# minhtrangvy/distributed_bitcoin_minter

Measured on AMD Instinct MI355X. Metric: GH/s (SHA-256 "msg nonce" min-search) at 1/2/4/8 MI355X; % of int32 VALU peak, higher is better.
Workload: dtype u32

## Files before the change

distributed_bitcoin_minter_amd/csrc/bm_kernels.hpp:

```cpp
#pragma once
#include <hip/hip_runtime.h>

#include <cstdint>
#include <type_traits>

#include "bm_common.h"
#include "bm_sha256.hpp"

namespace bm {

#define BM_DEV __device__ __forceinline__

template <int B, int E, class F>
BM_DEV void static_for(F&& f) {
    if constexpr (B < E) {
        f(std::integral_constant<int, B>{});
        static_for<B + 1, E>(f);
    }
}

BM_DEV uint32_t rotr(uint32_t x, uint32_t n) { return __builtin_amdgcn_alignbit(x, x, n); }

BM_DEV uint32_t xor3(uint32_t a, uint32_t b, uint32_t c) {
    if (__builtin_constant_p(a) && __builtin_constant_p(b) && __builtin_constant_p(c)) return a ^ b ^ c;
    return __builtin_amdgcn_bitop3_b32(a, b, c, 0x96);
}
BM_DEV uint32_t ch(uint32_t e, uint32_t f, uint32_t g) {
    if (__builtin_constant_p(e) && __builtin_constant_p(f) && __builtin_constant_p(g)) return (e & f) ^ (~e & g);
    return __builtin_amdgcn_bitop3_b32(e, f, g, 0xCA);
}
BM_DEV uint32_t maj(uint32_t a, uint32_t b, uint32_t c) {
    if (__builtin_constant_p(a) && __builtin_constant_p(b) && __builtin_constant_p(c))
        return (a & b) ^ (a & c) ^ (b & c);
    return __builtin_amdgcn_bitop3_b32(a, b, c, 0xE8);
}
BM_DEV uint32_t bsig0(uint32_t a) { return xor3(rotr(a, 2), rotr(a, 13), rotr(a, 22)); }
BM_DEV uint32_t bsig1(uint32_t e) { return xor3(rotr(e, 6), rotr(e, 11), rotr(e, 25)); }
BM_DEV uint32_t ssig0(uint32_t x) { return xor3(rotr(x, 7), rotr(x, 18), x >> 3); }
BM_DEV uint32_t ssig1(uint32_t x) { return xor3(rotr(x, 17), rotr(x, 19), x >> 10); }

template <int T>
BM_DEV void sha_round(uint32_t (&s)[8], uint32_t w) {
    uint32_t& a = s[(0 - T) & 7];
    uint32_t& b = s[(1 - T) & 7];
    uint32_t& c = s[(2 - T) & 7];
    uint32_t& d = s[(3 - T) & 7];
    uint32_t& e = s[(4 - T) & 7];
    uint32_t& f = s[(5 - T) & 7];
    uint32_t& g = s[(6 - T) & 7];
    uint32_t& h = s[(7 - T) & 7];
    const uint32_t t1 = h + bsig1(e) + ch(e, f, g) + (kK256[T] + w);
    d += t1;
    h = t1 + bsig0(a) + maj(a, b, c);
}

#ifndef BM_PAD_ADD3S
#define BM_PAD_ADD3S 1
#endif

BM_DEV uint32_t add3_sgpr(uint32_t a, uint32_t s, uint32_t b) {
    uint32_t r;
    asm("v_add3_u32 %0, %1, %2, %3" : "=v"(r) : "v"(a), "s"(s), "v"(b));
    return r;
}

template <int T, bool KW_SGPR = false>
BM_DEV void sha_round_kw(uint32_t (&s)[8], uint32_t kw) {
    uint32_t& a = s[(0 - T) & 7];
    uint32_t& b = s[(1 - T) & 7];
    uint32_t& c = s[(2 - T) & 7];
    uint32_t& d = s[(3 - T) & 7];
    uint32_t& e = s[(4 - T) & 7];
    uint32_t& f = s[(5 - T) & 7];
    uint32_t& g = s[(6 - T) & 7];
    uint32_t& h = s[(7 - T) & 7];
    uint32_t t1;
    if constexpr (KW_SGPR && BM_PAD_ADD3S)
        t1 = add3_sgpr(h, kw, ch(e, f, g)) + bsig1(e);
    else
        t1 = h + bsig1(e) + ch(e, f, g) + kw;
    d += t1;
    h = t1 + bsig0(a) + maj(a, b, c);
}

template <int R0, int R1>
BM_DEV void sha_rounds(uint32_t (&s)[8], uint32_t (&w)[16]) {
    static_for<R0, R1>([&](auto I) {
        constexpr int t = decltype(I)::value;
        if constexpr (t >= 16)
            w[t & 15] = ssig1(w[(t - 2) & 15]) + w[(t - 7) & 15] + ssig0(w[(t - 15) & 15]) + w[t & 15];
        sha_round<t>(s, w[t & 15]);
    });
}

BM_DEV uint32_t ssig0_uniform(uint32_t x) {
    return ((x >> 7) | (x << 25)) ^ ((x >> 18) | (x << 14)) ^ (x >> 3);
}

#ifndef BM_PIN
#define BM_PIN 1
#endif

BM_DEV uint32_t ssig0_salu(uint32_t x) {
    uint32_t r, t0, t1, t2;
    asm("s_lshr_b32 %1, %4, 7\n\t"
        "s_lshl_b32 %2, %4, 25\n\t"
        "s_or_b32 %1, %1, %2\n\t"
        "s_lshr_b32 %2, %4, 18\n\t"
        "s_lshl_b32 %3, %4, 14\n\t"
        "s_or_b32 %2, %2, %3\n\t"
        "s_xor_b32 %1, %1, %2\n\t"
        "s_lshr_b32 %2, %4, 3\n\t"
        "s_xor_b32 %0, %1, %2"
        : "=s"(r), "=&s"(t0), "=&s"(t1), "=&s"(t2)
        : "s"(x)
        : "scc");
    return r;
}

BM_DEV uint32_t vgpr_copy(uint32_t x) {
    uint32_t r;
    asm("v_mov_b32 %0, %1" : "=v"(r) : "s"(x));
    return r;
}

template <int R0, int V>
BM_DEV uint32_t sha_rounds_h0(uint32_t (&s)[8], uint32_t (&w)[16], uint32_t s0v, uint32_t h0_add) {
    static_assert(R0 <= V && V >= 1 && V <= 15, "varying word");
    static_for<R0, 63>([&](auto I) {
        constexpr int t = decltype(I)::value;
        if constexpr (t >= 16) {
            uint32_t s0;
            if constexpr (t - 15 == V)
                s0 = s0v;
            else
                s0 = ssig0(w[(t - 15) & 15]);
            w[t & 15] = ssig1(w[(t - 2) & 15]) + w[(t - 7) & 15] + s0 + w[t & 15];
        }
        sha_round<t>(s, w[t & 15]);
    });
    w[15] = ssig1(w[13]) + w[8] + ssig0(w[0]) + w[15];
    const uint32_t a = s[1], b = s[2], c = s[3], e = s[5], f = s[6], g = s[7], h = s[0];
    const uint32_t t1 = h + bsig1(e) + ch(e, f, g) + (kK256[63] + h0_add) + w[15];
    return t1 + bsig0(a) + maj(a, b, c);
}

BM_DEV void sha_compress(uint32_t (&st)[8], uint32_t (&w)[16]) {
    uint32_t s[8];
#pragma unroll
    for (int i = 0; i < 8; ++i) s[i] = st[i];
    sha_rounds<0, 64>(s, w);
#pragma unroll
    for (int i = 0; i < 8; ++i) st[i] += s[i];
}

template <int P, bool PADB>
constexpr int64_t tail_word(int k) {
    constexpr int LW = P / 4;
    if (k == LW + 1 && (P % 4) == 3 && P != 63) return 0x80000000ll;
    if (!PADB && k == 15) return -1;
    return 0;
}

template <int P, int NBV>
BM_DEV void add_task_digits(uint32_t (&W)[16 * NBV], uint64_t t, uint32_t ms, uint32_t nd) {
    uint64_t x = t;
    static_for<1, 20>([&](auto I) {
        constexpr int i = decltype(I)::value;
        constexpr int pos = 64 * (NBV - 1) + P - i;
        if constexpr (pos >= 0) {
            if (i >= (int)ms && i < (int)nd) {
                const uint64_t q = x / 10u;
                const uint32_t d = (uint32_t)(x - q * 10u);
                x = q;
                W[pos >> 2] += d << (8 * (3 - (pos & 3)));
            }
        }
    });
}

BM_DEV bool lex_less(uint64_t h1, uint64_t n1, uint64_t h2, uint64_t n2) {
    return h1 < h2 || (h1 == h2 && n1 < n2);
}

template <int XOR>
BM_DEV uint64_t swizzle_xor_u64(uint64_t v) {
    constexpr int pat = (XOR << 10) | 0x1F;
    const uint32_t lo = (uint32_t)__builtin_amdgcn_ds_swizzle((int)(uint32_t)v, pat);
    const uint32_t hi = (uint32_t)__builtin_amdgcn_ds_swizzle((int)(uint32_t)(v >> 32), pat);
    return ((uint64_t)hi << 32) | lo;
}

BM_DEV uint64_t readlane_u64(uint64_t v, int lane) {
    const uint32_t lo = (uint32_t)__builtin_amdgcn_readlane((int)(uint32_t)v, lane);
    const uint32_t hi = (uint32_t)__builtin_amdgcn_readlane((int)(uint32_t)(v >> 32), lane);
    return ((uint64_t)hi << 32) | lo;
}

BM_DEV void wave_min(uint64_t& h, uint64_t& n) {
    static_for<0, 5>([&](auto I) {
        constexpr int x = 1 << decltype(I)::value;
        const uint64_t oh = swizzle_xor_u64<x>(h), on = swizzle_xor_u64<x>(n);
        if (lex_less(oh, on, h, n)) {
            h = oh;
            n = on;
        }
    });
    const uint64_t h0 = readlane_u64(h, 0), n0 = readlane_u64(n, 0);
    const uint64_t h1 = readlane_u64(h, 32), n1 = readlane_u64(n, 32);
    if (lex_less(h1, n1, h0, n0)) {
        h = h1;
        n = n1;
    } else {
        h = h0;
        n = n0;
    }
}

template <int NT>
BM_DEV bool block_min(uint64_t& h, uint64_t& n) {
    constexpr int NWAVE = NT / 64;
    __shared__ Partial sh[NWAVE];
    wave_min(h, n);
    const int wave = threadIdx.x >> 6;
    if ((threadIdx.x & 63) == 0) sh[wave] = Partial{h, n};
    __syncthreads();
    if (threadIdx.x == 0) {
#pragma unroll
        for (int i = 1; i < NWAVE; ++i)
            if (lex_less(sh[i].hash, sh[i].nonce, h, n)) {
                h = sh[i].hash;
                n = sh[i].nonce;
            }
        return true;
    }
    return false;
}

BM_DEV uint64_t readfirstlane_u64(uint64_t v) {
    const uint32_t lo = (uint32_t)__builtin_amdgcn_readfirstlane((int)(uint32_t)v);
    const uint32_t hi = (uint32_t)__builtin_amdgcn_readfirstlane((int)(uint32_t)(v >> 32));
    return ((uint64_t)hi << 32) | lo;
}

#ifndef BM_FOLD
#define BM_FOLD 1
#endif
#ifndef BM_WAVES_MAIN
#define BM_WAVES_MAIN 7
#endif
#ifndef BM_WAVES_PAD
#define BM_WAVES_PAD 5
#endif
#ifndef BM_WAVES_NBV2
#define BM_WAVES_NBV2 7
#endif
#ifndef BM_NBV2_TIGHT
#define BM_NBV2_TIGHT 1
#endif
constexpr bool nbv2_tight(int P) { return BM_NBV2_TIGHT && P == 4; }
constexpr int search_waves(int P, int NBV) {
    return (NBV == 1 && P >= 55) ? BM_WAVES_PAD
                                 : (NBV == 2 ? (nbv2_tight(P) ? 6 : BM_WAVES_NBV2) : BM_WAVES_MAIN);
}
#ifndef BM_LDS_BEST
#define BM_LDS_BEST 0
#endif
#ifndef BM_CLOCK_PROBE
#define BM_CLOCK_PROBE 0
#endif
constexpr int kClockSlot = 16;
#ifndef BM_KATTR
#define BM_KATTR __attribute__((amdgpu_waves_per_eu(search_waves(P, NBV), 8)))
#endif

template <int P, int NBV, int PADK, bool TGT = false, bool HITS = false>
BM_DEV void search_body(const SearchArgs& A, Partial* __restrict__ part, unsigned long long* __restrict__ counter,
                        uint64_t target = 0, unsigned long long* hit = nullptr, Partial* hit_buf = nullptr,
                        uint64_t hit_cap = 0) {
    static_assert(!(TGT || HITS) || PADK == -1, "target and hits modes run the generic kernels");
    static_assert(!(TGT && HITS), "one mode");
    static_assert(P >= 0 && P < 64 && (NBV == 1 || (NBV == 2 && P <= 18)), "layout");
    constexpr int LW = P / 4;
    constexpr int BOFF = 16 * (NBV - 1);
    constexpr bool PADB = (NBV == 1) && (P >= 55);
    constexpr bool PADC = PADK >= 0;
    static_assert(!PADC || (PADB && PADK <= kMaxPadPrefixBlocks), "PADK is a padding-block layout");
    constexpr bool TWOW = (P % 4 == 0) && (LW >= 1);
    constexpr bool kFold = BM_FOLD && !PADB && LW >= 1 && !(NBV == 1 && (P == 53 || P == 54)) &&
                           !(NBV == 2 && P >= 17);
    constexpr bool kPin = BM_PIN && kFold && !(NBV == 1 && P >= 48);

    constexpr uint32_t inc0 = 1u << (8 * (3 - P % 4));
    constexpr uint32_t inc1 = (P % 4) >= 1 ? 1u << (8 * (4 - P % 4)) : 0u;
    constexpr uint32_t inc2 = (P % 4) >= 2 ? 1u << (8 * (5 - P % 4)) : 0u;
    constexpr uint32_t inc3 = (P % 4) >= 3 ? 1u << (8 * (6 - P % 4)) : 0u;

    uint64_t best_h = ~0ull, best_n = ~0ull;
    uint32_t bh = 0xFFFFFFFFu;
    const uint32_t thi = (uint32_t)(target >> 32);
    (void)thi;
#if BM_LDS_BEST
    __shared__ uint64_t lbest_h[kBlock], lbest_n[kBlock];
    lbest_h[threadIdx.x] = ~0ull;
    lbest_n[threadIdx.x] = ~0ull;
#endif

    const uint32_t S = A.S;
    const uint32_t n_in = TWOW ? 10u : S;
    const uint32_t n_out = TWOW ? S / 10u : 1u;
    const uint32_t lane = threadIdx.x & 63;
    const uint64_t ntask = A.t_end - A.t0;
    const uint64_t chunk = 64ull * A.chunk_m;

    if (BM_CLOCK_PROBE && blockIdx.x == 0 && threadIdx.x == 0) {
        counter[kClockSlot + 0] = __builtin_amdgcn_s_memtime();
        counter[kClockSlot + 1] = __builtin_amdgcn_s_memrealtime();
    }
    for (;;) {
        uint64_t base = 0;
        if constexpr (TGT) {
            uint64_t seen = 0;
            if (lane == 0) {
                base = atomicAdd(counter, (unsigned long long)chunk);
                seen = __hip_atomic_load(hit, __ATOMIC_RELAXED, __HIP_MEMORY_SCOPE_AGENT);
            }
            base = readfirstlane_u64(base);
            if (base >= ntask) break;
            seen = readfirstlane_u64(seen);
            if (seen < A.nonce_base || seen - A.nonce_base < (A.t0 + base) * (uint64_t)S) break;
        } else {
            if (lane == 0) base = atomicAdd(counter, (unsigned long long)chunk);
            base = readfirstlane_u64(base);
            if (base >= ntask) break;
        }
        for (uint32_t i = 0; i < A.chunk_m; ++i) {
            const uint64_t tt = base + 64ull * i + lane;
            if (tt >= ntask) break;
            const uint64_t t = A.t0 + tt;

            uint32_t W[16 * NBV];
            static_for<0, 16 * NBV>([&](auto K) { W[decltype(K)::value] = A.tmpl[decltype(K)::value]; });
            add_task_digits<P, NBV>(W, t, A.ms, A.nd);

            uint32_t st[8];
#pragma unroll
            for (int q = 0; q < 8; ++q) st[q] = PADK == 0 ? kIV256[q] : A.mid[q];
            if constexpr (NBV == 2) {
                uint32_t wa[16];
#pragma unroll
                for (int k = 0; k < 16; ++k) wa[k] = W[k];
                sha_compress(st, wa);
            }

            uint32_t wb[16];
            static_for<0, 16>([&](auto K) {
                constexpr int k = decltype(K)::value;
                if constexpr (k <= LW) {
                    wb[k] = W[BOFF + k];
                } else {
                    constexpr int64_t c = tail_word<P, PADB>(k);
                    if constexpr (c < 0)
                        wb[k] = (kPin && NBV == 1) ? vgpr_copy(A.tmpl[BOFF + k]) : A.tmpl[BOFF + k];
                    else
                        wb[k] = (uint32_t)c;
                }
            });
            constexpr int R0 = TWOW ? LW - 1 : LW;
            uint32_t s00[8];
#pragma unroll
            for (int q = 0; q < 8; ++q) s00[q] = st[q];
            sha_rounds<0, R0>(s00, wb);

            const uint64_t vbase = t * (uint64_t)S;
            for (uint32_t jo = 0; jo < n_out; ++jo) {
                uint32_t wo[16];
#pragma unroll
                for (int k = 0; k < 16; ++k) wo[k] = wb[k];
                uint32_t s0[8];
#pragma unroll
                for (int q = 0; q < 8; ++q) s0[q] = s00[q];
                if constexpr (TWOW) {
                    wo[LW - 1] = wb[LW - 1] + jo;
                    sha_rounds<LW - 1, LW>(s0, wo);
                }
                const uint32_t wl = wo[LW];
                const uint32_t s0wl = ssig0(wl);
                const uint32_t h0_add = (kPin && NBV == 1) ? vgpr_copy(st[0]) : st[0];
                const uint32_t h1_add = (kPin && NBV == 1) ? vgpr_copy(st[1]) : st[1];

                uint32_t J = 0, c0 = 0, c1 = 0, c2 = 0;
                for (uint32_t j = 0; j < n_in; ++j) {
                    uint32_t w[16];
#pragma unroll
                    for (int k = 0; k < 16; ++k) w[k] = wo[k];
                    w[LW] = wl + J;
                    uint32_t x[8];
#pragma unroll
                    for (int q = 0; q < 8; ++q) x[q] = s0[q];

                    uint32_t h0, h1;
                    if constexpr (kFold) {
                        const uint32_t s0J = kPin ? ssig0_salu(J) : ssig0_uniform(J);
                        h0 = sha_rounds_h0<LW, LW>(x, w, s0wl ^ s0J, h0_add);
                        h1 = h1_add + x[1];
                    } else if constexpr (PADB) {
                        sha_rounds<LW, 64>(x, w);
                        uint32_t y[8];
#pragma unroll
                        for (int q = 0; q < 8; ++q) y[q] = st[q] + x[q];
                        uint32_t z[8];
#pragma unroll
                        for (int q = 0; q < 8; ++q) z[q] = y[q];
                        static_for<0, 64>([&](auto I) {
                            constexpr int tt2 = decltype(I)::value;
                            if constexpr (PADC) {
                                constexpr uint32_t kw = kPadKW<P, (PADK > 0 ? PADK : 0)>.v[tt2];
                                sha_round_kw<tt2>(z, kw);
                            } else {
                                sha_round_kw<tt2, true>(z, A.padkw[tt2]);
                            }
                        });
                        h0 = y[0] + z[0];
                        h1 = y[1] + z[1];
                    } else {
                        sha_rounds<LW, 64>(x, w);
                        h0 = st[0] + x[0];
                        h1 = st[1] + x[1];
                    }

                    if (__builtin_expect(h0 <= bh, 0)) {
                        const uint64_t h = ((uint64_t)h0 << 32) | h1;
                        const uint64_t v = vbase + (uint64_t)jo * n_in + j;
                        if constexpr (TGT) {
                            if (h <= target && v >= A.vlo && v <= A.vhi)
                                atomicMin(hit, (unsigned long long)(A.nonce_base + v));
                        }
                        if constexpr (HITS) {
                            if (h <= target && v >= A.vlo && v <= A.vhi) {
                                const unsigned long long idx = atomicAdd(hit, 1ull);
                                if (idx < hit_cap) {
                                    using u64x2 = unsigned long long __attribute__((ext_vector_type(2)));
                                    *reinterpret_cast<u64x2*>(hit_buf + idx) = u64x2{h, A.nonce_base + v};
                                }
                            }
                        }
#if BM_LDS_BEST
                        if (h < lbest_h[threadIdx.x] && v >= A.vlo && v <= A.vhi) {
                            lbest_h[threadIdx.x] = h;
                            lbest_n[threadIdx.x] = A.nonce_base + v;
                            bh = HITS ? (h0 > thi ? h0 : thi) : h0;
                        }
#else
                        if (h < best_h && v >= A.vlo && v <= A.vhi) {
                            best_h = h;
                            best_n = A.nonce_base + v;
                            bh = HITS ? (h0 > thi ? h0 : thi) : h0;
                        }
#endif
                    }

                    J += inc0;
                    if (++c0 == 10u) {
                        c0 = 0;
                        J += inc1 - 10u * inc0;
                        if (++c1 == 10u) {
                            c1 = 0;
                            J += inc2 - 10u * inc1;
                            if (++c2 == 10u) {
                                c2 = 0;
                                J += inc3 - 10u * inc2;
                            }
                        }
                    }
                }
            }
        }
    }

    if (BM_CLOCK_PROBE && blockIdx.x == 0 && threadIdx.x == 0) {
        counter[kClockSlot + 2] = __builtin_amdgcn_s_memtime();
        counter[kClockSlot + 3] = __builtin_amdgcn_s_memrealtime();
    }
#if BM_LDS_BEST
    best_h = lbest_h[threadIdx.x];
    best_n = lbest_n[threadIdx.x];
#endif
    if (block_min<kBlock>(best_h, best_n)) part[A.part_off + blockIdx.x] = Partial{best_h, best_n};
}

template <int P, int NBV>
__global__ __launch_bounds__(kBlock) BM_KATTR void search_kernel(
    const SearchArgs A, Partial* __restrict__ part, unsigned long long* __restrict__ counter) {
    search_body<P, NBV, -1>(A, part, counter);
}

template <int P, int NBV = 1>
__global__ __launch_bounds__(kBlock) BM_KATTR void search_kernel_padc(
    const SearchArgs A, Partial* __restrict__ part, unsigned long long* __restrict__ counter) {
    static_assert(NBV == 1 && P >= 55, "padding-block layouts only");
    search_body<P, 1, 0>(A, part, counter);
}

template <int P, int K, int NBV = 1>
__global__ __launch_bounds__(kBlock) BM_KATTR void search_kernel_padk(
    const SearchArgs A, Partial* __restrict__ part, unsigned long long* __restrict__ counter) {
    static_assert(NBV == 1 && P >= 55 && K >= 1 && K <= kMaxPadPrefixBlocks, "padding-block layouts only");
    search_body<P, 1, K>(A, part, counter);
}

template <int P, int NBV>
__global__ __launch_bounds__(kBlock) BM_KATTR void target_kernel(
    const SearchArgs A, Partial* __restrict__ part, unsigned long long* __restrict__ counter, const uint64_t target,
    unsigned long long* __restrict__ hit) {
    search_body<P, NBV, -1, true>(A, part, counter, target, hit);
}

template <int P, int NBV>
__global__ __launch_bounds__(kBlock) BM_KATTR void hits_kernel(
    const SearchArgs A, Partial* __restrict__ part, unsigned long long* __restrict__ counter, const uint64_t target,
    unsigned long long* __restrict__ hit_count, Partial* __restrict__ hit_buf, const uint64_t hit_cap) {
    search_body<P, NBV, -1, false, true>(A, part, counter, target, hit_count, hit_buf, hit_cap);
}

}
```

Baseline: 55.17.

## Replace per-task decimal digit division with incremental packed-BCD addition held in LDS

Instead of producing each task's ASCII decimal digits through repeated 64-bit divisions by 10 per thread, each lane now converts the chunk base once. It then keeps its packed digit words in LDS and advances them by 64 per iteration with a SWAR decimal-add that propagates carries. The nonce index is rebuilt from the chunk base plus the lane offset. This removes the costly 64-bit division chain from the outer loop, at the cost of LDS traffic and extra per-chunk setup. A constexpr layout predicate limits it to some template configurations.

```diff
diff --git a/distributed_bitcoin_minter_amd/csrc/bm_kernels.hpp b/distributed_bitcoin_minter_amd/csrc/bm_kernels.hpp
--- a/distributed_bitcoin_minter_amd/csrc/bm_kernels.hpp
+++ b/distributed_bitcoin_minter_amd/csrc/bm_kernels.hpp
@@ -6,6 +6,7 @@
 
 #include "bm_common.h"
 #include "bm_sha256.hpp"
+#include "bm_task_digits.hpp"
 
 namespace bm {
 
@@ -179,6 +180,23 @@
     });
 }
 
+#ifndef BM_TASK_INCR
+#define BM_TASK_INCR 1
+#endif
+constexpr bool task_incr_layout(int P, int NBV, int PADK, bool TGT, bool HITS) {
+    if (NBV == 1 && PADK == -1 && !TGT && (P <= 2 || P == 4 || (!HITS && P >= 8 && P <= 11) || (HITS && P >= 5 && P <= 6)))
+        return false;
+    if (PADK == 0 && P == 60) return false;
+    return true;
+}
+
+BM_DEV uint32_t lds_get(const uint32_t* p) {
+    return __hip_atomic_load(p, __ATOMIC_RELAXED, __HIP_MEMORY_SCOPE_WORKGROUP);
+}
+BM_DEV void lds_put(uint32_t* p, uint32_t v) {
+    __hip_atomic_store(p, v, __ATOMIC_RELAXED, __HIP_MEMORY_SCOPE_WORKGROUP);
+}
+
 BM_DEV bool lex_less(uint64_t h1, uint64_t n1, uint64_t h2, uint64_t n2) {
     return h1 < h2 || (h1 == h2 && n1 < n2);
 }
@@ -313,6 +331,14 @@
     const uint64_t ntask = A.t_end - A.t0;
     const uint64_t chunk = 64ull * A.chunk_m;
 
+    constexpr bool kIncr = BM_TASK_INCR != 0 && task_incr_layout(P, NBV, PADK, TGT, HITS);
+    constexpr int NW = task_digit_words(P, NBV);
+    __shared__ uint32_t ldig[kIncr ? NW + 2 : 1][kBlock];
+    if constexpr (kIncr) {
+        lds_put(&ldig[NW][threadIdx.x], (A.ms + 3 - P % 4) | (A.nd + 3 - P % 4) << 8);
+        lds_put(&ldig[NW + 1][threadIdx.x], (uint32_t)small_addend(lane, 0));
+    }
+
     if (BM_CLOCK_PROBE && blockIdx.x == 0 && threadIdx.x == 0) {
         counter[kClockSlot + 0] = __builtin_amdgcn_s_memtime();
         counter[kClockSlot + 1] = __builtin_amdgcn_s_memrealtime();
@@ -334,14 +360,51 @@
             base = readfirstlane_u64(base);
             if (base >= ntask) break;
         }
+        if constexpr (kIncr) {
+            const uint32_t g0 = (uint32_t)__builtin_amdgcn_readfirstlane((int)lds_get(&ldig[NW][threadIdx.x])) & 0xFFu;
+            uint32_t U[NW];
+            chunk_digits<NW>(U, A.t0 + base, g0);
+            const uint64_t lane_add = (uint64_t)lds_get(&ldig[NW + 1][threadIdx.x]) << (8 * g0);
+            uint32_t carry = 0;
+            static_for<0, NW>([&](auto K) {
+                constexpr int k = decltype(K)::value;
+                lds_put(&ldig[k][threadIdx.x], dec_add_word(U[k], dec_addend_word(lane_add, k), carry));
+            });
+        }
         for (uint32_t i = 0; i < A.chunk_m; ++i) {
-            const uint64_t tt = base + 64ull * i + lane;
-            if (tt >= ntask) break;
-            const uint64_t t = A.t0 + tt;
+            const uint64_t tu = base + 64ull * i;
+            uint64_t t = 0;
+            if constexpr (kIncr) {
+                const uint32_t left = tu >= ntask ? 0u : (ntask - tu > 64u ? 64u : (uint32_t)(ntask - tu));
+                if (lane >= left) break;
+            } else {
+                const uint64_t tt = tu + lane;
+                if (tt >= ntask) break;
+                t = A.t0 + tt;
+            }
 
             uint32_t W[16 * NBV];
             static_for<0, 16 * NBV>([&](auto K) { W[decltype(K)::value] = A.tmpl[decltype(K)::value]; });
-            add_task_digits<P, NBV>(W, t, A.ms, A.nd);
+            if constexpr (kIncr) {
+                const uint32_t cfg = (uint32_t)__builtin_amdgcn_readfirstlane((int)lds_get(&ldig[NW][threadIdx.x]));
+                const uint32_t g0 = cfg & 0xFFu, glim = cfg >> 8;
+                uint32_t D[NW];
+                static_for<0, NW>([&](auto K) {
+                    constexpr int k = decltype(K)::value;
+                    D[k] = lds_get(&ldig[k][threadIdx.x]);
+                    W[BOFF + LW - k] = (D[k] & digit_mask(k, glim)) | A.tmpl[BOFF + LW - k];
+                });
+                if (i + 1 < A.chunk_m) {
+                    const uint64_t step = small_addend(64u, g0);
+                    uint32_t carry = 0;
+                    static_for<0, NW>([&](auto K) {
+                        constexpr int k = decltype(K)::value;
+                        lds_put(&ldig[k][threadIdx.x], dec_add_word(D[k], dec_addend_word(step, k), carry));
+                    });
+                }
+            } else {
+                add_task_digits<P, NBV>(W, t, A.ms, A.nd);
+            }
 
             uint32_t st[8];
 #pragma unroll
@@ -372,7 +435,7 @@
             for (int q = 0; q < 8; ++q) s00[q] = st[q];
             sha_rounds<0, R0>(s00, wb);
 
-            const uint64_t vbase = t * (uint64_t)S;
+            const uint64_t vbase = (kIncr ? A.t0 + tu : t) * (uint64_t)S;
             for (uint32_t jo = 0; jo < n_out; ++jo) {
                 uint32_t wo[16];
 #pragma unroll
@@ -431,7 +494,8 @@
 
                     if (__builtin_expect(h0 <= bh, 0)) {
                         const uint64_t h = ((uint64_t)h0 << 32) | h1;
-                        const uint64_t v = vbase + (uint64_t)jo * n_in + j;
+                        const uint64_t v =
+                            kIncr ? vbase + (lane * S + jo * n_in + j) : vbase + (uint64_t)jo * n_in + j;
                         if constexpr (TGT) {
                             if (h <= target && v >= A.vlo && v <= A.vhi)
                                 atomicMin(hit, (unsigned long long)(A.nonce_base + v));
diff --git a/distributed_bitcoin_minter_amd/csrc/bm_task_digits.hpp b/distributed_bitcoin_minter_amd/csrc/bm_task_digits.hpp
--- /dev/null
+++ b/distributed_bitcoin_minter_amd/csrc/bm_task_digits.hpp
@@ -0,0 +1,72 @@
+#pragma once
+#include <cstdint>
+
+#if defined(__HIPCC__)
+#define BM_TD __host__ __device__ __forceinline__
+#else
+#define BM_TD inline
+#endif
+
+namespace bm {
+
+constexpr int task_digit_words(int P, int NBV) {
+    const int imax = (64 * (NBV - 1) + P) < 19 ? (64 * (NBV - 1) + P) : 19;
+    return (imax + 3 - P % 4) / 4 + 1;
+}
+
+BM_TD uint32_t dec_add_word(uint32_t a, uint32_t b, uint32_t& carry) {
+    const uint32_t t = a + b + carry;
+    const uint32_t u = t + 0xF6F6F6F6u;
+    const uint32_t co = ~u & 0x80808080u;
+    carry = co >> 31;
+    return t + (co << 1) - (co >> 4) - (co >> 6);
+}
+
+template <int NW>
+BM_TD void chunk_digits(uint32_t (&U)[NW], uint64_t c, uint32_t g0) {
+    uint32_t V[7] = {0, 0, 0, 0, 0, 0, 0};
+    uint64_t x = c;
+#if defined(__HIP_DEVICE_COMPILE__)
+#pragma unroll
+#endif
+    for (int j = 0; j < 20; ++j) {
+        const uint64_t q = x / 10u;
+        V[j >> 2] |= (uint32_t)(x - q * 10u) << (8 * (j & 3));
+        x = q;
+    }
+    const uint32_t ws = g0 >> 2, bs = 8 * (g0 & 3);
+#if defined(__HIP_DEVICE_COMPILE__)
+#pragma unroll
+#endif
+    for (int k = 0; k < NW; ++k) {
+        const uint32_t hi = ws ? (k >= 1 ? V[k - 1] : 0u) : V[k];
+        const uint32_t lo = ws ? (k >= 2 ? V[k - 2] : 0u) : (k >= 1 ? V[k - 1] : 0u);
+        U[k] = (uint32_t)(((((uint64_t)hi << 32) | lo) << bs) >> 32);
+    }
+}
+
+BM_TD uint64_t small_addend(uint32_t x, uint32_t g0) {
+    const uint32_t q = (x * 205u) >> 11;
+    return (uint64_t)(x + 246u * q) << (8 * g0);
+}
+
+BM_TD uint32_t dec_addend_word(uint64_t add, int k) {
+    return k == 0 ? (uint32_t)add : k == 1 ? (uint32_t)(add >> 32) : 0u;
+}
+
+template <int NW>
+BM_TD void dec_add(uint32_t (&U)[NW], uint64_t add) {
+    uint32_t carry = 0;
+#if defined(__HIP_DEVICE_COMPILE__)
+#pragma unroll
+#endif
+    for (int k = 0; k < NW; ++k)
+        U[k] = dec_add_word(U[k], dec_addend_word(add, k), carry);
+}
+
+BM_TD uint32_t digit_mask(int k, uint32_t glim) {
+    const int n = (int)glim - 4 * k;
+    return n >= 4 ? 0xFFFFFFFFu : n <= 0 ? 0u : (1u << (8 * n)) - 1u;
+}
+
+}
```

Measured after the change: 55.30, median of 6. No clear change (+0.2%).
